# LCJebe/PCReg

Measured on AMD Instinct MI355X. Metric: KNN Gpairs/s end-to-end (search + filters + RANSAC per step; registrations/s = 1000/ms_per_step), higher is better.
Workload: dtype f32 (search: f16-split matrix-core candidates, exact f32 re-rank) / f64 (RANSAC)

## Files before the change

### include/pcreg.h

```cpp
#ifndef PCREG_H
#define PCREG_H
#include <stddef.h>
#include <stdint.h>

#ifdef __cplusplus
extern "C" {
#endif

#define PCREG_OK            0
#define PCREG_E_ARG         1
#define PCREG_E_HIP         2
#define PCREG_E_NODEVICE    3
#define PCREG_E_WORKSPACE   4

#define PCREG_KNN_MAX_K 32

#define PCREG_METRIC_SAD 0
#define PCREG_METRIC_SSD 1

typedef struct pcreg_ransac_opts {
    int32_t  minPtNum;
    int32_t  iterNum;
    double   thDist;
    double   thInlrRatio;
    int32_t  REFINE;
    int32_t  VERBOSE;
    uint64_t seed;
} pcreg_ransac_opts;

typedef struct pcreg_match_opts {
    int32_t metric;
    double  matchThreshold;
    double  maxRatio;
    int32_t unique;
    int32_t prenormalized;
    int32_t unnormalize;
    double  norm_factor;
    int32_t change_metric;
    double  metric_factor;
} pcreg_match_opts;

const char* pcreg_last_error(void);
const char* pcreg_version(void);
int  pcreg_device_count(int* count);
int  pcreg_set_device(int ordinal);
int  pcreg_device_name(char* buf, int cap);
int  pcreg_debug_set(const char* key, int value);
int  pcreg_debug_match_stats(long long out[8], int reset);
int  pcreg_debug_knn_stats(long long out[4], int reset);
int  pcreg_debug_knn_unit_stats(long long out[2], int reset);
int  pcreg_debug_knn_direct_stats(long long out[3], int reset);
int  pcreg_debug_ransac_stats(long long out[3], int reset);
int  pcreg_debug_cluster_stats(long long out[4], int reset);
int  pcreg_debug_desc_stats(long long out[10], int reset);


int pcreg_estimate_transform(const double* pts1, const double* pts2, int n, int ld,
                             double T[16], int* empty);

int pcreg_calc_dists(const double T[16], const double* pts1, const double* pts2, int n, int ld,
                     double* d);

int pcreg_ransac(const double* pts1, const double* pts2, int n, int ld,
                 const pcreg_ransac_opts* opts, const int32_t* sample_idx,
                 double T[16], int32_t* inlier_idx, int* n_inliers, int* num_success,
                 int* max_inliers, int* failed, int32_t* iter_inl, int32_t* iter_inl_ref);

int pcreg_ransac_batched(const double* pts1, const double* pts2, int total, int ld,
                         const int32_t* offsets, int B, const pcreg_ransac_opts* opts,
                         const int32_t* sample_idx, double* T, int32_t* inlier_idx,
                         int32_t* n_inliers, int32_t* num_success, int32_t* max_inliers,
                         int32_t* failed);

int pcreg_knn2_points_f32(const float* q, int Q, int ldq, const float* m, int M, int ldm,
                          int32_t* idx, float* dist);

int pcreg_match_points_f32(const float* q, int Q, int ldq, const float* m, int M, int ldm,
                           float thr_abs, float max_ratio, int unique,
                           uint32_t* pairs, int* P);

typedef struct pcreg_model pcreg_model;
int pcreg_model_create(const float* m, int M, int ldm, pcreg_model** model);
int pcreg_model_destroy(pcreg_model* model);
int pcreg_model_size(const pcreg_model* model, int* M);
int pcreg_model_match_points_f32(pcreg_model* model, const float* q, int Q, int ldq, float thr_abs, float max_ratio,
// ... 429 lines not shown
```

### pcreg_amd/_lib.py

```python
from __future__ import annotations

import ctypes as C
import os

_HERE = os.path.dirname(os.path.abspath(__file__))
LIB_PATH = os.environ.get("PCREG_LIB") or os.path.join(_HERE, "libpcreg_hip.so")

PCREG_OK, PCREG_E_ARG, PCREG_E_HIP, PCREG_E_NODEVICE, PCREG_E_WORKSPACE = 0, 1, 2, 3, 4
KNN_MAX_K = 32
METRIC_SAD, METRIC_SSD = 0, 1
LAYOUT_FEATURE_MAJOR, LAYOUT_ROW_MAJOR = 0, 1


class PcregError(RuntimeError):
    def __init__(self, code: int, msg: str):
        super().__init__(f"libpcreg_hip error {code}: {msg}")
        self.code = code


class RansacOpts(C.Structure):
    _fields_ = [("minPtNum", C.c_int32), ("iterNum", C.c_int32), ("thDist", C.c_double),
                ("thInlrRatio", C.c_double), ("REFINE", C.c_int32), ("VERBOSE", C.c_int32),
                ("seed", C.c_uint64)]


class MatchOpts(C.Structure):
    _fields_ = [("metric", C.c_int32), ("matchThreshold", C.c_double), ("maxRatio", C.c_double),
                ("unique", C.c_int32), ("prenormalized", C.c_int32), ("unnormalize", C.c_int32),
                ("norm_factor", C.c_double), ("change_metric", C.c_int32), ("metric_factor", C.c_double)]


class DescOpts(C.Structure):
    _fields_ = [("min_pts", C.c_int32), ("max_pts", C.c_int32), ("R", C.c_double), ("thVar", C.c_double * 2),
                ("k", C.c_double), ("ALIGN_POINTS", C.c_int32)]


class DevRansacResult(C.Structure):
    _fields_ = [("T", C.c_double * 16), ("n_inliers", C.c_int32), ("num_success", C.c_int32),
                ("max_inliers", C.c_int32), ("failed", C.c_int32), ("n", C.c_int32), ("winner", C.c_int32)]


SYMBOLS = [
    "pcreg_last_error", "pcreg_version", "pcreg_device_count", "pcreg_set_device", "pcreg_device_name", "pcreg_debug_set", "pcreg_debug_match_stats",
    "pcreg_debug_knn_stats", "pcreg_debug_knn_unit_stats", "pcreg_debug_knn_direct_stats", "pcreg_debug_ransac_stats", "pcreg_debug_cluster_stats", "pcreg_debug_desc_stats", "pcreg_debug_dev_model_export", "pcreg_debug_search_export",
    "pcreg_estimate_transform", "pcreg_calc_dists", "pcreg_ransac", "pcreg_ransac_batched",
    "pcreg_knn2_points_f32", "pcreg_match_points_f32", "pcreg_match_features", "pcreg_get_matches", "pcreg_desc_set_create", "pcreg_desc_set_destroy", "pcreg_desc_set_size", "pcreg_get_matches_on_sets", "pcreg_get_matches_segmented_on_sets", "pcreg_sphere_counts", "pcreg_sphere_sweep", "pcreg_sphere_model_create", "pcreg_sphere_model_destroy", "pcreg_sphere_sweep_on_model", "pcreg_final_stage_limits", "pcreg_final_stage", "pcreg_get_matches_segmented", "pcreg_get_local_points",
    "pcreg_model_create", "pcreg_model_destroy", "pcreg_model_size", "pcreg_model_match_points_f32", "pcreg_model_knn_f32", "pcreg_knn_points_f32",
    "pcreg_model_range_f32", "pcreg_range_points_f32", "pcreg_model_cluster_f32", "pcreg_cluster_points_f32",
    "pcreg_dev_model_create", "pcreg_dev_model_destroy", "pcreg_dev_model_search_workspace", "pcreg_dev_model_search_f32",
    "pcreg_dev_model_knn_workspace", "pcreg_dev_model_knn_f32", "pcreg_dev_merge_topk_f32",
    "pcreg_dev_model_range_workspace", "pcreg_dev_model_range_count_f32", "pcreg_dev_model_range_fill_f32",
    "pcreg_dev_model_cluster_workspace", "pcreg_dev_model_cluster_f32",
    "pcreg_model_score_f32", "pcreg_dev_model_score_workspace", "pcreg_dev_model_score_f32",
    "pcreg_model_refit_f32", "pcreg_dev_model_refit_workspace", "pcreg_dev_model_refit_f32",
    "pcreg_model_normals_f32", "pcreg_point_normals_f32", "pcreg_dev_model_normals_workspace", "pcreg_dev_model_normals_f32",
    "pcreg_model_refit_plane_f32", "pcreg_dev_model_refit_plane_workspace", "pcreg_dev_model_refit_plane_f32",
    "pcreg_model_denoise_f32", "pcreg_point_denoise_f32", "pcreg_dev_model_denoise_workspace", "pcreg_dev_model_denoise_f32",
    "pcreg_model_fpfh_f32", "pcreg_point_fpfh_f32", "pcreg_dev_model_fpfh_workspace", "pcreg_dev_model_fpfh_f32",
    "pcreg_model_fpfh_radius_f32", "pcreg_point_fpfh_radius_f32", "pcreg_dev_model_fpfh_radius_workspace", "pcreg_dev_model_fpfh_radius_count_f32",
    "pcreg_dev_model_fpfh_radius_f32",
    "pcreg_model_iss_f32", "pcreg_point_iss_f32", "pcreg_dev_model_iss_workspace", "pcreg_dev_model_iss_f32",
    "pcreg_model_fit_planes_f32", "pcreg_point_fit_planes_f32", "pcreg_dev_model_fit_planes_workspace", "pcreg_dev_model_fit_planes_f32",
    "pcreg_model_fit_spheres_f32", "pcreg_point_fit_spheres_f32", "pcreg_dev_model_fit_spheres_workspace", "pcreg_dev_model_fit_spheres_f32",
    "pcreg_model_fit_cylinders_f32", "pcreg_point_fit_cylinders_f32", "pcreg_dev_model_fit_cylinders_workspace", "pcreg_dev_model_fit_cylinders_f32",
    "pcreg_unique_rows3", "pcreg_aggregate_matches", "pcreg_dev_unique_rows3_workspace", "pcreg_dev_unique_rows3_f64",
    "pcreg_dev_aggregate_matches_workspace", "pcreg_dev_aggregate_matches", "pcreg_dev_estimate_transform_indexed",
    "pcreg_downsample_grid_f32", "pcreg_dev_downsample_grid_workspace", "pcreg_dev_downsample_grid_chunk", "pcreg_dev_downsample_grid_f32",
    "pcreg_ndt_create", "pcreg_ndt_destroy", "pcreg_ndt_size", "pcreg_ndt_get", "pcreg_ndt_refit_f32",
    "pcreg_dev_ndt_create", "pcreg_dev_ndt_destroy", "pcreg_dev_ndt_size", "pcreg_dev_ndt_get", "pcreg_dev_ndt_refit_workspace", "pcreg_dev_ndt_refit_f32",
    "pcreg_dev_model_match_f32", "pcreg_dev_model_match_table_f32", "pcreg_dev_match_from_table_f32",
    "pcreg_align_points_knn", "pcreg_align_points_knn_f32", "pcreg_align_points_knn_batched", "pcreg_spatial_histogram_descriptors",
    "pcreg_spatial_histogram_descriptors_f32", "pcreg_spatial_histogram_descriptors_mixed",
    "pcreg_dev_knn2_points_f32_workspace", "pcreg_dev_knn2_points_f32", "pcreg_dev_merge_top2_f32", "pcreg_dev_merge_top2_strided_f32",
    "pcreg_dev_ransac_workspace", "pcreg_dev_ransac",
    "pcreg_dev_ransac_partial", "pcreg_dev_ransac_finish", "pcreg_dev_ransac_finish_parts",
    "pcreg_dev_search_kernel_timing", "pcreg_dev_search_kernel_ms",
    "pcreg_dev_spatial_histogram_descriptors_workspace", "pcreg_dev_spatial_histogram_descriptors",
# ... 122 lines not shown
            L.pcreg_dev_model_refit_plane_workspace.argtypes = [C.c_int] * 3
            vp, i, f = C.c_void_p, C.c_int, C.c_float
            L.pcreg_dev_model_refit_plane_f32.argtypes = [vp, vp, i, i, vp, i, f, vp, i, vp, vp, vp, vp, vp, vp, vp, vp, C.c_size_t, vp]
            L.pcreg_model_refit_plane_f32.argtypes = [vp, vp, i, i, vp, i, f, i, vp, i, i, vp, vp, vp, vp, vp, vp]
        if hasattr(L, "pcreg_dev_unique_rows3_workspace"):
            for name in ("pcreg_dev_unique_rows3_workspace", "pcreg_dev_aggregate_matches_workspace"):
                getattr(L, name).restype = C.c_size_t
                getattr(L, name).argtypes = [C.c_int]
        if hasattr(L, "pcreg_dev_downsample_grid_workspace"):
            L.pcreg_dev_downsample_grid_workspace.restype = C.c_size_t
            L.pcreg_dev_downsample_grid_workspace.argtypes = [C.c_int]
            L.pcreg_dev_downsample_grid_chunk.argtypes = []
            vp, i, d = C.c_void_p, C.c_int, C.c_double
            L.pcreg_dev_downsample_grid_f32.argtypes = [vp, i, i, d, vp, i, vp, vp, vp, vp, vp, C.c_size_t, vp]
            L.pcreg_downsample_grid_f32.argtypes = [vp, i, i, d, vp, i, vp, vp, vp]
        if hasattr(L, "pcreg_dev_ndt_refit_workspace"):
            L.pcreg_dev_ndt_refit_workspace.restype = C.c_size_t
            L.pcreg_dev_ndt_refit_workspace.argtypes = [C.c_int, C.c_int]
            vp, i, d = C.c_void_p, C.c_int, C.c_double
            L.pcreg_dev_ndt_create.argtypes = [vp, i, i, d, i, vp, vp]
            L.pcreg_ndt_create.argtypes = [vp, i, i, d, i, vp]
            for name in ("pcreg_dev_ndt_destroy", "pcreg_ndt_destroy"):
                getattr(L, name).argtypes = [vp]
            for name in ("pcreg_dev_ndt_size", "pcreg_ndt_size"):
                getattr(L, name).argtypes = [vp, vp, vp]
            for name in ("pcreg_dev_ndt_get", "pcreg_ndt_get"):
                getattr(L, name).argtypes = [vp] * 7
            L.pcreg_dev_ndt_refit_f32.argtypes = [vp, vp, i, i, vp, i, i, d, vp, vp, vp, vp, vp, vp, C.c_size_t, vp]
            L.pcreg_ndt_refit_f32.argtypes = [vp, vp, i, i, vp, i, i, d, i, vp, vp, vp, vp]
        for name, args in (("pcreg_debug_knn_stats", [C.POINTER(C.c_longlong), C.c_int]),
                           ("pcreg_debug_knn_unit_stats", [C.POINTER(C.c_longlong), C.c_int]),
                           ("pcreg_debug_knn_direct_stats", [C.POINTER(C.c_longlong), C.c_int]),
                           ("pcreg_debug_ransac_stats", [C.POINTER(C.c_longlong), C.c_int]),
                           ("pcreg_debug_desc_stats", [C.POINTER(C.c_longlong), C.c_int]),
                           ("pcreg_debug_dev_model_export", [C.c_void_p] * 4 + [C.POINTER(C.c_float), C.c_void_p]),
                           ("pcreg_debug_search_export", [C.c_void_p, C.c_size_t, C.c_int, C.c_int] + [C.c_void_p] * 3)):
            if hasattr(L, name):
                getattr(L, name).argtypes = args
        _lib = L
    return _lib


def check(rc: int) -> None:
    if rc != PCREG_OK:
        raise PcregError(rc, lib().pcreg_last_error().decode(errors="replace"))
```

### pcreg_amd/csrc/api.hip

```cpp
#include "common.hpp"
#include <atomic>
#include <cstdarg>
#include <cmath>
#include <mutex>
#include <algorithm>
#include <vector>

namespace pcreg {

static thread_local char g_err[512] = "no error";
void set_error(const char* fmt, ...) {
    va_list ap; va_start(ap, fmt);
    vsnprintf(g_err, sizeof g_err, fmt, ap);
    va_end(ap);
}

constexpr int kKnnMaxK = PCREG_KNN_MAX_K;
constexpr int kKnnMaxQ = 4 << 20;
constexpr int kRangeMaxQ = 4 << 20;
constexpr int kScoreMaxQ = 4 << 20;
static std::mutex g_mu;
static int g_device_ok = -1;
static hipStream_t g_stream = nullptr;

// ... 59 lines not shown
        if (hipMalloc((void**)&c.dev, c.n * sizeof(unsigned long long)) != hipSuccess) { c.dev = nullptr; return nullptr; }
        (void)hipMemset(c.dev, 0, c.n * sizeof(unsigned long long));
    }
    return c.dev;
}
static int counters_read(const Counters& c, long long* out, int reset, int first = 0, int count = -1) {
    PCREG_ARG(out != nullptr);
    if (count < 0) count = c.n - first;
    for (int k = 0; k < count; ++k) out[k] = 0;
    if (!c.dev) return PCREG_OK;
    PCREG_HIP(hipDeviceSynchronize());
    unsigned long long h[8];
    PCREG_HIP(hipMemcpy(h, c.dev + first, count * sizeof h[0], hipMemcpyDeviceToHost));
    for (int k = 0; k < count; ++k) out[k] = (long long)h[k];
    if (reset) PCREG_HIP(hipMemset(c.dev + first, 0, count * sizeof h[0]));
    return PCREG_OK;
}
unsigned long long* match_stats_dev() { return counters_dev(g_match_stats); }
unsigned long long* knn_stats_dev() { return counters_dev(g_knn_stats); }
unsigned long long* ransac_stats_dev() { return counters_dev(g_ransac_stats); }
unsigned long long* cluster_stats_dev() { return counters_dev(g_cluster_stats); }
unsigned long long* desc_stats_dev() { return counters_dev(g_desc_stats); }
unsigned long long* knn_direct_stats_dev() { return counters_dev(g_knn_direct_stats); }
}

extern "C" {

int pcreg_debug_set(const char* key, int value) {
    static const char* const names[pcreg::kDbgCount] = {"knn_exact", "match_exact", "match_force_fallback", "ransac_fused", "ransac_nolane",
                                                        "ransac_f64score", "ransac_resident_f64", "align_times", "align_shape", "seg_debug",
                                                        "seg_batched", "seg_wave_finalize", "match_stats", "final_batch_mb", "knn_nocull",
                                                        "knn_stats", "ransac_pass2", "ransac_stats", "range_sort_cap", "cluster_noskip",
                                                        "cluster_stats", "knn_tail_cap", "score_batch_slots", "fpfh_radius_lanes", "desc_stats",
                                                        "knn_direct", "knn_direct_stats", "knn_seed_fused"};
    PCREG_ARG(key != nullptr);
    for (int k = 0; k < pcreg::kDbgCount; ++k)
        if (!strcmp(key, names[k])) { pcreg::g_debug[k].store(value, std::memory_order_relaxed); return PCREG_OK; }
    pcreg::set_error("pcreg_debug_set: unknown key '%s'", key);
    return PCREG_E_ARG;
}

int pcreg_debug_match_stats(long long out[8], int reset) { return pcreg::counters_read(pcreg::g_match_stats, out, reset); }
int pcreg_debug_knn_stats(long long out[4], int reset) { return pcreg::counters_read(pcreg::g_knn_stats, out, reset, 0, 4); }
int pcreg_debug_knn_unit_stats(long long out[2], int reset) { return pcreg::counters_read(pcreg::g_knn_stats, out, reset, 4, 2); }
int pcreg_debug_knn_direct_stats(long long out[3], int reset) { return pcreg::counters_read(pcreg::g_knn_direct_stats, out, reset); }
int pcreg_debug_ransac_stats(long long out[3], int reset) { return pcreg::counters_read(pcreg::g_ransac_stats, out, reset); }
int pcreg_debug_cluster_stats(long long out[4], int reset) { return pcreg::counters_read(pcreg::g_cluster_stats, out, reset); }
int pcreg_debug_desc_stats(long long out[10], int reset) {
    PCREG_ARG(out != nullptr);
    TRY(pcreg::counters_read(pcreg::g_desc_stats, out, reset, 0, 8));
    return pcreg::counters_read(pcreg::g_desc_stats, out + 8, reset, 8, 2);
}

const char* pcreg_last_error(void) { return g_err; }
const char* pcreg_version(void) { return "pcreg-hip 0.1 (gfx950)"; }

int pcreg_device_count(int* count) {
    PCREG_ARG(count != nullptr);
    hipError_t e = hipGetDeviceCount(count);
    if (e != hipSuccess) { *count = 0; (void)hipGetLastError(); }
    return PCREG_OK;
}

static void*  g_pin[2] = {nullptr, nullptr};
static size_t g_pin_bytes[2] = {0, 0};
static hipEvent_t g_pairs_ev = nullptr;

int pcreg_set_device(int ordinal) {
    std::lock_guard<std::mutex> lock(g_mu);
    int count = 0;
    if (hipGetDeviceCount(&count) != hipSuccess || count <= 0) { set_error("no HIP device available"); (void)hipGetLastError(); return PCREG_E_NODEVICE; }
    PCREG_ARG(ordinal >= 0 && ordinal < count);
    scratch().release_all();
    if (g_stream) { (void)hipStreamDestroy(g_stream); g_stream = nullptr; }
    if (g_pairs_ev) { (void)hipEventDestroy(g_pairs_ev); g_pairs_ev = nullptr; }
    for (int k = 0; k < 2; ++k) if (g_pin[k]) { (void)hipHostFree(g_pin[k]); g_pin[k] = nullptr; g_pin_bytes[k] = 0; }
    g_device_ok = -1;
    PCREG_HIP(hipSetDevice(ordinal));
    return ensure_device();
// ... 2551 lines not shown
```

### pcreg_amd/csrc/common.hpp

```cpp
#pragma once
#include <cstdlib>
#include <hip/hip_runtime.h>
#include <cstdint>
#include <cstdio>
#include <cstring>
#include <algorithm>
#include <string>
#include "../../include/pcreg.h"

namespace pcreg {

void set_error(const char* fmt, ...);
int  ensure_device();

#define PCREG_HIP(call)                                                                  \
    do {                                                                                 \
        hipError_t e__ = (call);                                                         \
        if (e__ != hipSuccess) {                                                         \
            ::pcreg::set_error("%s failed: %s (%s:%d)", #call, hipGetErrorString(e__),   \
                               __FILE__, __LINE__);                                      \
            return PCREG_E_HIP;                                                          \
        }                                                                                \
    } while (0)

#define PCREG_ARG(cond)                                                                  \
    do {                                                                                 \
        if (!(cond)) {                                                                   \
            ::pcreg::set_error("bad argument: %s (%s:%d)", #cond, __FILE__, __LINE__);   \
            return PCREG_E_ARG;                                                          \
        }                                                                                \
    } while (0)

struct Scratch {
    static constexpr int kSlots = 24;
    void*  ptr[kSlots]  = {};
    size_t size[kSlots] = {};
    int get(int slot, size_t bytes, void** out);
    void release_all();
};
// ... 8 lines not shown
        return rc;
    }
};

enum DebugKey {
    kDbgKnnExact = 0,
    kDbgMatchExact,
    kDbgMatchForceFallback,
    kDbgRansacFused,
    kDbgRansacNoLane,
    kDbgRansacF64Score,
    kDbgRansacResidentF64,
    kDbgAlignTimes,
    kDbgAlignShape,
    kDbgSegDebug,
    kDbgSegBatched,
    kDbgSegWaveFinalize,
    kDbgMatchStats,
    kDbgFinalBatchMB,
    kDbgKnnNoCull,
    kDbgKnnStats,
    kDbgRansacPass2,
    kDbgRansacStats,
    kDbgRangeSortCap,
    kDbgClusterNoSkip,
    kDbgClusterStats,
    kDbgKnnTailCap,
    kDbgScoreBatchSlots,
    kDbgFpfhRadiusLanes,
    kDbgDescStats,
    kDbgKnnDirect,
    kDbgKnnDirectStats,
    kDbgKnnSeedFused,
    kDbgCount
};
int debug_flag(DebugKey k);
unsigned long long* match_stats_dev();
unsigned long long* knn_stats_dev();
unsigned long long* knn_direct_stats_dev();
unsigned long long* ransac_stats_dev();
unsigned long long* cluster_stats_dev();
unsigned long long* desc_stats_dev();
#ifdef PCREG_EXPERIMENTS
static inline int pcreg_env_int(const char* name, int dflt) { const char* e = getenv(name); return e ? atoi(e) : dflt; }
static inline const char* pcreg_env_str(const char* name) { return getenv(name); }
#define PCREG_EXP_ENV(name, dflt) pcreg_env_int(name, dflt)
#define PCREG_EXP_STR(name) pcreg_env_str(name)
#else
#define PCREG_EXP_ENV(name, dflt) (dflt)
#define PCREG_EXP_STR(name) ((const char*)nullptr)
#endif

static inline size_t align_up(size_t x, size_t a) { return (x + a - 1) / a * a; }

struct WsWalk {
    char* base; size_t off = 0;
    explicit WsWalk(void* b) : base((char*)b) {}
    void* take_bytes(size_t bytes) { void* p = base ? base + off : nullptr; off += bytes; return p; }
    template <class T> T* take(size_t count, size_t align = 256) { return (T*)take_bytes(align_up(count * sizeof(T), align)); }
    size_t bytes() const { return off; }
};

template <typename T>
static int upload_cols(const T* host, int n, int ld, int cols, T* dev, hipStream_t st) {
    if (n <= 0 || cols <= 0) return PCREG_OK;
    if (ld == n) { PCREG_HIP(hipMemcpyAsync(dev, host, sizeof(T) * (size_t)n * cols, hipMemcpyHostToDevice, st)); }
    else PCREG_HIP(hipMemcpy2DAsync(dev, sizeof(T) * (size_t)n, host, sizeof(T) * (size_t)ld, sizeof(T) * (size_t)n, cols, hipMemcpyHostToDevice, st));
    return PCREG_OK;
}

struct RansacDims { int n_cap; int iters; int B; };

size_t ransac_workspace_bytes(int iters, int B, int n_cap);
// ... 217 lines not shown
```

### pcreg_amd/csrc/ransac.hip

```cpp
#include "common.hpp"
#include "moments.hpp"
#include "wave_math.hpp"
#include <cfloat>
#include <cstddef>
#include <cstdio>
#include <cstdlib>

namespace pcreg {
namespace {

constexpr int kBlock = 256;
constexpr int kWavesPerBlock = 4;
constexpr int HB = 4;

struct RansacArgs {
    const double* p1; const double* p2; int ld;
    const int32_t* offsets;
    const int32_t* n_dev;
    int n_cap; int iters; int m;
    double thDist; double ratio; int refine; unsigned long long seed;
    const int32_t* sample_idx;
    int hpw;
    int hyp0g;
    double* TF;
// ... 1324 lines not shown
                cnt += __popcll(b[s]);                                                                             \
                if (EMIT) {                                                               \
                    asm volatile("v_writelane_b32 %0, %1, %2" : "+v"(mine_lo) : "s"((int)(unsigned)b[s]), "n"(s)); \
                    asm volatile("v_writelane_b32 %0, %1, %2" : "+v"(mine_hi) : "s"((int)(unsigned)(b[s] >> 32)), "n"(s)); \
                }                                                                                                  \
            }                                                                                                      \
            if (lane == 0) s_cnt[wave][(H) - h0] += cnt;                                                           \
            if (EMIT && lane < kSS)                            \
                sa.masks[(size_t)(H) * sa.nslots_cap + (size_t)pb * (kSPts / 64) + wave * kSS + lane] =            \
                    ((unsigned long long)(unsigned)mine_hi << 32) | (unsigned)mine_lo;                             \
        }
        PCREG_ROW_LOAD(RA, h0)
        PCREG_ROW_WAIT(RA);
        for (int h = h0; h < h1; h += 2) {
            PCREG_ROW_LOAD(RB, h + 1)
            PCREG_SCORE_HYP(h, RA)
            PCREG_ROW_WAIT(RB); PCREG_ROW_LOAD(RA, h + 2)
            if (h + 1 < h1) { PCREG_SCORE_HYP(h + 1, RB) }
            PCREG_ROW_WAIT(RA);
        }
#undef PCREG_SCORE_HYP
#undef PCREG_ROW_WAIT
#undef PCREG_ROW_LOAD
    }
    __syncthreads();
    for (int hl = threadIdx.x; hl < h1 - h0; hl += kSW * 64) {
        int c = 0;
#pragma unroll
        for (int w = 0; w < kSW; ++w) c += s_cnt[w][hl];
        if (acc) { if (c) atomicAdd(&acc[h0 + hl], c); } else sa.part[(size_t)blockIdx.x * a.iters + h0 + hl] = c;
    }
}


__device__ __forceinline__ void rs_load_block(const StagedArgs& sa, const float* __restrict__ x32, int base, int n, float (&q)[kSS][6]) {
    const int lane = threadIdx.x & 63;
#pragma unroll
    for (int s = 0; s < kSS; ++s) {
        const int i = base + s * 64 + lane;
        const bool act = i < n;
        const int ii = act ? i : 0;
#pragma unroll
        for (int c = 0; c < 6; ++c) q[s][c] = x32[(size_t)c * sa.n32 + ii];
        if (!act) q[s][0] = __builtin_nanf("");
    }
}
__device__ __forceinline__ int rs_block_count(const StagedArgs& sa, const float* __restrict__ x32, const int32_t* __restrict__ perm,
                                              int base, int n, const float (&q)[kSS][6], const float (&T)[12], float thlo, float thhi,
                                              int h) {
    const RansacArgs& a = sa.a;
    const int lane = threadIdx.x & 63;
    unsigned long long b[kSS], band = 0ull;
#pragma unroll
    for (int s = 0; s < kSS; ++s) {
        const float d = sqdist32(q[s], T);
        b[s] = __ballot(d < thlo);
        band |= __ballot(d <= thhi) ^ b[s];
    }
    if (band != 0ull && !PCREG_NOBAND(sa)) {
        double T64[12];
#pragma unroll
        for (int k = 0; k < 12; ++k) T64[k] = a.TF[(size_t)h * 12 + k];
#pragma unroll 1
        for (int s = 0; s < kSS; ++s) {
            const int i = base + s * 64 + lane;
            const bool act = i < n;
// ... 1477 lines not shown
            double tv = 0.0;
#pragma unroll
            for (int e = 0; e < 12; ++e) if (e == j * 4 + k) tv = T[e];
            v = (j < 3) ? tv : (k == 3 ? 1.0 : 0.0);
        }
        s_S[k + 4 * j] = v;
        if (T_step) T_step[(size_t)bl * 16 + k + 4 * j] = v;
    }
    __builtin_amdgcn_fence(__ATOMIC_ACQ_REL, "wavefront"); __builtin_amdgcn_wave_barrier();
    if (lane < 16) {
        const int r = lane & 3, c = lane >> 2;
        const double* Ti = T_in + (size_t)bl * 16;
        const double v = ((Ti[r] * s_S[4 * c] + Ti[r + 4] * s_S[1 + 4 * c]) + Ti[r + 8] * s_S[2 + 4 * c]) + Ti[r + 12] * s_S[3 + 4 * c];
        T_out[(size_t)bl * 16 + r + 4 * c] = ok ? v : 0.0;
    }
    if (lane == 0) empty[bl] = ok ? 0 : 1;
}

__global__ void calc_dists_kernel(const double* T16, const double* p1, const double* p2, int n, int ld, double* d) {
    double T[12];
#pragma unroll
    for (int j = 0; j < 3; ++j)
#pragma unroll
        for (int k = 0; k < 4; ++k) T[j * 4 + k] = T16[k + 4 * j];
    Pts<false> P{p1, p2, ld, nullptr, n};
    for (int i = blockIdx.x * blockDim.x + threadIdx.x; i < n; i += gridDim.x * blockDim.x) {
        double q[6]; P.load(i, q);
        d[i] = sqdist(q, T);
    }
}

}

static bool staged_pays(int n_cap, int iters) { return n_cap >= 4096 || (n_cap >= kStagedMinN && (long long)n_cap * iters >= 20000000LL); }
static bool bounded_pays(int n_cap, int iters) {
    const double full_us = (double)n_cap * (double)iters / 2.4e6, bounded_us = 1.4 * (double)((n_cap + kBBlk - 1) / kBBlk) + 30.0;
    return full_us > 1.1 * bounded_us;
}
static size_t staged_slots_cap(int n_cap) { return (size_t)((n_cap + kSPts - 1) / kSPts) * (kSPts / 64); }
static size_t staged_chunks_cap(int n_cap) { return (staged_slots_cap(n_cap) + kMomSlots - 1) / kMomSlots; }
struct RansacWs { double* TF; int32_t* cnt1; int32_t* cnt2; unsigned char* has; double* msc; StagedArgs sa; };
static RansacWs ransac_ws_layout(int iters, int B, int n_cap, void* base, size_t* bytes) {
    const size_t h = (size_t)iters * (size_t)B;
    const int nc = B == 1 ? n_cap : 0;
    const size_t slots = staged_slots_cap(nc);
    WsWalk w(base);
    RansacWs s{};
    StagedArgs& sa = s.sa;
    s.TF = w.take<double>(h * 12);
    s.cnt1 = w.take<int32_t>(h); s.cnt2 = w.take<int32_t>(h);
    s.has = w.take<unsigned char>(h); s.msc = w.take<double>(h * 16);
    sa.T1 = w.take<double>(h * 12); sa.mom = w.take<double>(h * 27);
    sa.part = w.take<int32_t>(h * kSMaxPB);
    sa.v1 = w.take<unsigned char>(h); sa.pass1 = w.take<unsigned char>(h); sa.v2 = w.take<unsigned char>(h);
    sa.cert = w.take<unsigned char>(h); sa.dense = w.take<unsigned char>(h);
    sa.bounds = (double*)w.take_bytes(256);
    sa.n_rec_blocks = (int)((slots * 64 + 255) / 256);
    sa.bpart = w.take<double>((size_t)sa.n_rec_blocks * 4);
    sa.sel_ctr = w.take_bytes(512);
    sa.certq = w.take<double>(h * 2);
    if (nc >= kStagedMinN) {
        sa.nslots_cap = (int)slots;
        sa.masks = w.take<unsigned long long>(h * slots);
        sa.rec = w.take<double>(slots * 64 * kRec + 32);
        sa.mpart = w.take<double>(staged_chunks_cap(nc) * h * 15);
        sa.pass_list = w.take<int32_t>(h);
        sa.dig = w.take<uint4>(slots * 2 * 256);
        sa.n_pass = (int32_t*)w.take_bytes(256);
        sa.n32 = (int)slots * 64;
        sa.c32 = w.take<float>((size_t)sa.n32 * 6);
// ... 59 lines not shown
        const int c = n_cap <= kHyp32Classes[0] ? 0 : 1;
        a.n_lo = -1; a.n_hi = std::min(n_cap, kHyp32Classes[c]);
        const int nw = kHyp32Waves[c], per_block = hpw * nw;
        const dim3 grid((o.iterNum + per_block - 1) / per_block, B);
        const int rc = nw == 8 ? launch_hyp32<8>(a, grid, hyp32_lds_bytes(a.n_hi, nw), st) : launch_hyp32<16>(a, grid, hyp32_lds_bytes(a.n_hi, nw), st);
        if (rc != PCREG_OK) return rc;
        const int lo = a.n_hi;
        if (n_cap > lo) {
            a.n_lo = lo; a.n_hi = -1;
            const int pb4 = hpw * kWavesPerBlock;
            hipLaunchKernelGGL(ransac_hyp_kernel, dim3((o.iterNum + pb4 - 1) / pb4, B), dim3(kBlock), 0, st, a);
        }
    } else if (B == 1 && !offsets && staged_pays(n_cap, o.iterNum) && !debug_flag(kDbgRansacFused)) {
        StagedArgs sa = lay.sa;
        sel_ctr = sa.sel_ctr;
        sa.use_lane = a.refine && !debug_flag(kDbgRansacNoLane);
        sa.use_f32 = !debug_flag(kDbgRansacF64Score);
#ifdef PCREG_EXPERIMENTS
        sa.noband = PCREG_EXP_ENV("PCREG_RANSAC_NOBAND", 0);
#endif
        int pb = (n_cap + kSPts - 1) / kSPts; if (pb > kSMaxPB) pb = kSMaxPB; if (pb < 1) pb = 1;
        sa.pb = pb;
        int hpw = (int)((total + 250LL * kTW - 1) / (250LL * kTW));
        if (hpw < 1) hpw = 1;
        if (hpw > 16) hpw = 16;
        a.hpw = hpw;
        sa.a = a;
        const int it = o.iterNum;
        const dim3 sgrid(pb, (it + kSChunk - 1) / kSChunk);
        const int n_fit = (it + 255) / 256;
        hipLaunchKernelGGL(rs_stage1_kernel, dim3((unsigned)(n_fit + sa.n_rec_blocks)), dim3(256), 0, st, sa, n_fit);
        const int n_t32 = (it + 255) / 256, n_dig = sa.use_lane ? (int)staged_slots_cap(n_cap) * 2 : 0;
        hipLaunchKernelGGL(rs_stage2_kernel, dim3((unsigned)(n_t32 + n_dig)), dim3(256), 0, st, sa, (const double*)sa.T1, sa.T32a, n_t32, sa.dig);
        if (sa.use_f32) {
            if (sa.use_lane)
                hipLaunchKernelGGL(rs_score32_kernel<true>, sgrid, dim3(kSW * 64), 0, st, sa, (const double*)sa.T1, (const float*)sa.T32a, (const unsigned char*)sa.v1, (int32_t*)nullptr);
            else
                hipLaunchKernelGGL(rs_score32_kernel<false>, sgrid, dim3(kSW * 64), 0, st, sa, (const double*)sa.T1, (const float*)sa.T32a, (const unsigned char*)sa.v1, (int32_t*)nullptr);
        } else if (sa.use_lane) {
            hipLaunchKernelGGL(rs_score_kernel<true>, sgrid, dim3(kSW * 64), 0, st, sa, (const double*)sa.T1, (const unsigned char*)sa.v1);
        } else {
            hipLaunchKernelGGL(rs_score_kernel<false>, sgrid, dim3(kSW * 64), 0, st, sa, (const double*)sa.T1, (const unsigned char*)sa.v1);
        }
        hipLaunchKernelGGL(rs_pass1_kernel, dim3((it + 255) / 256), dim3(256), 0, st, sa);
        if (a.refine) {
            if (sa.use_lane)
                hipLaunchKernelGGL(rs_moments_mfma_kernel, dim3((it + kMmWaves * kMmRows - 1) / (kMmWaves * kMmRows), (unsigned)staged_chunks_cap(n_cap)), dim3(kMmWaves * 64), 0, st, sa,
                                   (const uint4*)sa.dig, (const unsigned long long*)sa.masks);
            hipLaunchKernelGGL(rs_moments_kernel, dim3((it + hpw * kTW - 1) / (hpw * kTW)), dim3(kTBlock), 0, st, sa);
            hipLaunchKernelGGL(rs_fit2_kernel, dim3((it + 63) / 64), dim3(64), 0, st, sa);
            fold_finish = !part && n_cap <= kSelBlocks * kSelPerThread * kSelThreads;
            const int p2mode = debug_flag(kDbgRansacPass2);
            const bool bounded = fold_finish && sa.use_f32 && !iter_inl_ref && p2mode != 1 && (p2mode == 2 || bounded_pays(n_cap, it));
            if (bounded) {
                const int S = std::min(kBSeeds, it), nbc = (n_cap + kBBlk - 1) / kBBlk;
                const int n_seed_wg = (S * nbc + 3) / 4, n_ord_wg = (n_cap + 255) / 256;
                unsigned long long* stats = ransac_stats_dev();
                hipLaunchKernelGGL(rs_bprep_kernel, dim3((unsigned)(n_seed_wg + n_ord_wg)), dim3(256), 0, st, sa, n_seed_wg, S, nbc);
                hipLaunchKernelGGL(rs_bscatter_kernel, dim3((unsigned)n_ord_wg), dim3(256), 0, st, sa);
#ifdef PCREG_EXPERIMENTS
                const int dbg = PCREG_EXP_ENV("PCREG_RANSAC_DEBUG", 0), chunk = PCREG_EXP_ENV("PCREG_RANSAC_BCHUNK", kBChunk);
                unsigned long long* kst = dbg ? ((BCtr*)sa.bctr)->stats : stats;
                if (chunk == 8) hipLaunchKernelGGL(rs_bounded_kernel<8>, dim3((unsigned)((it + 7) / 8)), dim3(64), 0, st, sa, kst);
                else if (chunk == 2) hipLaunchKernelGGL(rs_bounded_kernel<2>, dim3((unsigned)((it + 1) / 2)), dim3(64), 0, st, sa, kst);
                else hipLaunchKernelGGL(rs_bounded_kernel<kBChunk>, dim3((unsigned)((it + kBChunk - 1) / kBChunk)), dim3(64), 0, st, sa, kst);
                if (dbg) {
                    unsigned long long u[3] = {0, 0, 0};
                    PCREG_HIP(hipMemcpyAsync(u, kst, sizeof u, hipMemcpyDeviceToHost, st));
                    PCREG_HIP(hipStreamSynchronize(st));
                    fprintf(stderr, "[pcreg] ransac bounded pass 2: iters=%d n_cap=%d chunk=%d (refit, block) units scanned %llu of %llu (%.4f)\n", it, n_cap,
                            chunk == 8 || chunk == 2 ? chunk : kBChunk, u[1], u[2], u[2] ? (double)u[1] / (double)u[2] : 0.0);
                }
#else
                hipLaunchKernelGGL(rs_bounded_kernel<kBChunk>, dim3((unsigned)((it + kBChunk - 1) / kBChunk)), dim3(64), 0, st, sa, stats);
#endif
            } else if (sa.use_f32)
                hipLaunchKernelGGL(rs_score32_kernel<false>, sgrid, dim3(kSW * 64), 0, st, sa, (const double*)a.TF, (const float*)sa.T32b, (const unsigned char*)sa.v2,
                                   fold_finish ? a.cnt2 : (int32_t*)nullptr);
            else
                hipLaunchKernelGGL(rs_score_kernel<false>, sgrid, dim3(kSW * 64), 0, st, sa, (const double*)a.TF, (const unsigned char*)sa.v2);
            if (fold_finish) { sel_fin.part = sa.use_f32 ? nullptr : sa.part; sel_fin.v2 = sa.v2; sel_fin.pb = sa.pb; }
            else hipLaunchKernelGGL(rs_finish_kernel, dim3((it + 255) / 256), dim3(256), 0, st, sa);
        }
    } else {
        int hpw = (int)((total + 250LL * kTW - 1) / (250LL * kTW));
        if (hpw < 1) hpw = 1;
        if (hpw > 16) hpw = 16;
        a.hpw = hpw;
        int per_block = hpw * kTW;
        dim3 grid((o.iterNum + per_block - 1) / per_block, B);
        hipLaunchKernelGGL(ransac_hyp_tiled_kernel, grid, dim3(kTBlock), 0, st, a);
    }
    PCREG_HIP(hipGetLastError());
    if (sel_ctr && !part && n_cap <= kSelBlocks * kSelPerThread * kSelThreads) {
        int per_block = 4 * kSelThreads;
        if ((n_cap + per_block - 1) / per_block > kSelBlocks) per_block = ((n_cap + kSelBlocks - 1) / kSelBlocks + kSelThreads - 1) / kSelThreads * kSelThreads;
        const int nb = std::max(1, (n_cap + per_block - 1) / per_block);
        hipLaunchKernelGGL(ransac_select_multi_kernel, dim3(nb), dim3(kSelThreads), 0, st, a, out, inlier_idx, (SelCtr*)sel_ctr, per_block, sel_fin);
    }
    else if (n_cap >= 8192) hipLaunchKernelGGL(ransac_select_kernel<1024>, dim3(B), dim3(1024), 0, st, a, out, inlier_idx, part);
    else hipLaunchKernelGGL(ransac_select_kernel<kBlock>, dim3(B), dim3(kBlock), 0, st, a, out, inlier_idx, part);
    PCREG_HIP(hipGetLastError());
    if (iter_inl) PCREG_HIP(hipMemcpyAsync(iter_inl, a.cnt1, h * sizeof(int32_t), hipMemcpyDeviceToDevice, st));
    if (iter_inl_ref) PCREG_HIP(hipMemcpyAsync(iter_inl_ref, a.cnt2, h * sizeof(int32_t), hipMemcpyDeviceToDevice, st));
    return PCREG_OK;
}

int launch_ransac(const double* p1, const double* p2, int ld, const int32_t* offsets, const int32_t* n_dev,
                  int n_cap, int B, const pcreg_ransac_opts& o, const int32_t* sample_idx_dev,
                  pcreg_dev_ransac_result* out, int32_t* inlier_idx, int32_t* iter_inl, int32_t* iter_inl_ref,
                  void* ws, size_t ws_bytes, hipStream_t st) {
    return launch_ransac_impl(p1, p2, ld, offsets, n_dev, n_cap, B, o, sample_idx_dev, out, inlier_idx, iter_inl, iter_inl_ref,
                              ws, ws_bytes, st, 0, nullptr);
}

// ... 73 lines not shown
```

Baseline: 142,600.

## Add hypothesis-per-lane RANSAC scoring kernel with LDS-staged points and ballot masks

Adds rs_hscore_kernel, where each lane owns one RANSAC hypothesis and the workgroup stages 512 points in shared memory. Each lane tests every staged point with an inline-asm f32 transform-distance routine, builds inlier bitmasks from low/high band thresholds via ballots, and resolves ambiguous band points with an exact f64 check. The kernel is meant to replace rs_score32_kernel when the workgroup count is large enough, for both the first scoring pass and the pass-2 rescoring. It aims to raise data reuse and cut per-point work. The trade-offs are higher register pressure and a divergent f64 fallback loop.

```diff
diff --git a/include/pcreg.h b/include/pcreg.h
--- a/include/pcreg.h
+++ b/include/pcreg.h
@@ -51,6 +51,7 @@
 int  pcreg_debug_knn_unit_stats(long long out[2], int reset);
 int  pcreg_debug_knn_direct_stats(long long out[3], int reset);
 int  pcreg_debug_ransac_stats(long long out[3], int reset);
+int  pcreg_debug_ransac_score_stats(long long out[2], int reset);
 int  pcreg_debug_cluster_stats(long long out[4], int reset);
 int  pcreg_debug_desc_stats(long long out[10], int reset);
 
diff --git a/pcreg_amd/_lib.py b/pcreg_amd/_lib.py
--- a/pcreg_amd/_lib.py
+++ b/pcreg_amd/_lib.py
@@ -42,7 +42,7 @@
 
 SYMBOLS = [
     "pcreg_last_error", "pcreg_version", "pcreg_device_count", "pcreg_set_device", "pcreg_device_name", "pcreg_debug_set", "pcreg_debug_match_stats",
-    "pcreg_debug_knn_stats", "pcreg_debug_knn_unit_stats", "pcreg_debug_knn_direct_stats", "pcreg_debug_ransac_stats", "pcreg_debug_cluster_stats", "pcreg_debug_desc_stats", "pcreg_debug_dev_model_export", "pcreg_debug_search_export",
+    "pcreg_debug_knn_stats", "pcreg_debug_knn_unit_stats", "pcreg_debug_knn_direct_stats", "pcreg_debug_ransac_stats", "pcreg_debug_ransac_score_stats", "pcreg_debug_cluster_stats", "pcreg_debug_desc_stats", "pcreg_debug_dev_model_export", "pcreg_debug_search_export",
     "pcreg_estimate_transform", "pcreg_calc_dists", "pcreg_ransac", "pcreg_ransac_batched",
     "pcreg_knn2_points_f32", "pcreg_match_points_f32", "pcreg_match_features", "pcreg_get_matches", "pcreg_desc_set_create", "pcreg_desc_set_destroy", "pcreg_desc_set_size", "pcreg_get_matches_on_sets", "pcreg_get_matches_segmented_on_sets", "pcreg_sphere_counts", "pcreg_sphere_sweep", "pcreg_sphere_model_create", "pcreg_sphere_model_destroy", "pcreg_sphere_sweep_on_model", "pcreg_final_stage_limits", "pcreg_final_stage", "pcreg_get_matches_segmented", "pcreg_get_local_points",
     "pcreg_model_create", "pcreg_model_destroy", "pcreg_model_size", "pcreg_model_match_points_f32", "pcreg_model_knn_f32", "pcreg_knn_points_f32",
@@ -231,6 +231,7 @@
                            ("pcreg_debug_knn_unit_stats", [C.POINTER(C.c_longlong), C.c_int]),
                            ("pcreg_debug_knn_direct_stats", [C.POINTER(C.c_longlong), C.c_int]),
                            ("pcreg_debug_ransac_stats", [C.POINTER(C.c_longlong), C.c_int]),
+                           ("pcreg_debug_ransac_score_stats", [C.POINTER(C.c_longlong), C.c_int]),
                            ("pcreg_debug_desc_stats", [C.POINTER(C.c_longlong), C.c_int]),
                            ("pcreg_debug_dev_model_export", [C.c_void_p] * 4 + [C.POINTER(C.c_float), C.c_void_p]),
                            ("pcreg_debug_search_export", [C.c_void_p, C.c_size_t, C.c_int, C.c_int] + [C.c_void_p] * 3)):
diff --git a/pcreg_amd/csrc/api.hip b/pcreg_amd/csrc/api.hip
--- a/pcreg_amd/csrc/api.hip
+++ b/pcreg_amd/csrc/api.hip
@@ -115,7 +115,7 @@
                                                         "seg_batched", "seg_wave_finalize", "match_stats", "final_batch_mb", "knn_nocull",
                                                         "knn_stats", "ransac_pass2", "ransac_stats", "range_sort_cap", "cluster_noskip",
                                                         "cluster_stats", "knn_tail_cap", "score_batch_slots", "fpfh_radius_lanes", "desc_stats",
-                                                        "knn_direct", "knn_direct_stats", "knn_seed_fused"};
+                                                        "knn_direct", "knn_direct_stats", "knn_seed_fused", "ransac_score"};
     PCREG_ARG(key != nullptr);
     for (int k = 0; k < pcreg::kDbgCount; ++k)
         if (!strcmp(key, names[k])) { pcreg::g_debug[k].store(value, std::memory_order_relaxed); return PCREG_OK; }
@@ -128,6 +128,11 @@
 int pcreg_debug_knn_unit_stats(long long out[2], int reset) { return pcreg::counters_read(pcreg::g_knn_stats, out, reset, 4, 2); }
 int pcreg_debug_knn_direct_stats(long long out[3], int reset) { return pcreg::counters_read(pcreg::g_knn_direct_stats, out, reset); }
 int pcreg_debug_ransac_stats(long long out[3], int reset) { return pcreg::counters_read(pcreg::g_ransac_stats, out, reset); }
+int pcreg_debug_ransac_score_stats(long long out[2], int reset) {
+    PCREG_ARG(out != nullptr);
+    for (int k = 0; k < 2; ++k) out[k] = reset ? pcreg::g_ransac_score_launches[k].exchange(0) : pcreg::g_ransac_score_launches[k].load();
+    return PCREG_OK;
+}
 int pcreg_debug_cluster_stats(long long out[4], int reset) { return pcreg::counters_read(pcreg::g_cluster_stats, out, reset); }
 int pcreg_debug_desc_stats(long long out[10], int reset) {
     PCREG_ARG(out != nullptr);
diff --git a/pcreg_amd/csrc/common.hpp b/pcreg_amd/csrc/common.hpp
--- a/pcreg_amd/csrc/common.hpp
+++ b/pcreg_amd/csrc/common.hpp
@@ -5,6 +5,7 @@
 #include <cstdio>
 #include <cstring>
 #include <algorithm>
+#include <atomic>
 #include <string>
 #include "../../include/pcreg.h"
 
@@ -79,6 +80,7 @@
     kDbgKnnDirect,
     kDbgKnnDirectStats,
     kDbgKnnSeedFused,
+    kDbgRansacScore,
     kDbgCount
 };
 int debug_flag(DebugKey k);
@@ -86,6 +88,7 @@
 unsigned long long* knn_stats_dev();
 unsigned long long* knn_direct_stats_dev();
 unsigned long long* ransac_stats_dev();
+extern std::atomic<long long> g_ransac_score_launches[2];
 unsigned long long* cluster_stats_dev();
 unsigned long long* desc_stats_dev();
 #ifdef PCREG_EXPERIMENTS
diff --git a/pcreg_amd/csrc/ransac.hip b/pcreg_amd/csrc/ransac.hip
--- a/pcreg_amd/csrc/ransac.hip
+++ b/pcreg_amd/csrc/ransac.hip
@@ -1380,6 +1380,153 @@
     }
 }
 
+__device__ __forceinline__ void push_bit(unsigned& own, unsigned long long ballot);
+__device__ __forceinline__ float sqdist32v(const float4& q, const float2& r, const float (&T)[12]) {
+    float tx, ty, tz, d;
+    asm("v_fma_f32 %0, %9, %12, %19\n\t"
+        "v_fma_f32 %1, %9, %15, %20\n\t"
+        "v_fma_f32 %2, %9, %18, %21\n\t"
+        "v_fma_f32 %0, %8, %11, %0\n\t"
+        "v_fma_f32 %1, %8, %14, %1\n\t"
+        "v_fma_f32 %2, %8, %17, %2\n\t"
+        "v_fma_f32 %0, %7, %10, %0\n\t"
+        "v_fma_f32 %1, %7, %13, %1\n\t"
+        "v_fma_f32 %2, %7, %16, %2\n\t"
+        "v_sub_f32 %0, %4, %0\n\t"
+        "v_sub_f32 %1, %5, %1\n\t"
+        "v_sub_f32 %2, %6, %2\n\t"
+        "v_mul_f32 %3, %0, %0\n\t"
+        "v_fma_f32 %3, %1, %1, %3\n\t"
+        "v_fma_f32 %3, %2, %2, %3"
+        : "=&v"(tx), "=&v"(ty), "=&v"(tz), "=&v"(d)
+        : "v"(q.x), "v"(q.y), "v"(q.z), "v"(q.w), "v"(r.x), "v"(r.y),
+          "v"(T[0]), "v"(T[1]), "v"(T[2]), "v"(T[3]), "v"(T[4]), "v"(T[5]), "v"(T[6]), "v"(T[7]), "v"(T[8]),
+          "v"(T[9]), "v"(T[10]), "v"(T[11]));
+    return d;
+}
+constexpr int kHPts = 512, kHW = 4, kHWords = kHPts / 32;
+typedef unsigned rs_u32x16 __attribute__((ext_vector_type(16)));
+static_assert(kHWords == 16 && kSPts % kHPts == 0, "a lane's words are one rs_u32x16; the blocks tile rs_score32_kernel's");
+template <bool EMIT>
+__global__ __launch_bounds__(kHW * 64) void rs_hscore_kernel(StagedArgs sa, const double* __restrict__ TT,
+                                                             const float* __restrict__ T32,
+                                                             const unsigned char* __restrict__ valid,
+                                                             int32_t* __restrict__ acc ) {
+    const RansacArgs& a = sa.a;
+    __shared__ float4 s_rec[kHPts * 2];
+    const int n = staged_n(a);
+    const int h = blockIdx.y * (kHW * 64) + threadIdx.x;
+    const int hc = min(h, a.iters - 1);
+    const bool live = h < a.iters && valid[hc] != 0;
+    float T[12], thlo, thhi;
+    {
+        const float4* rp = (const float4*)(T32 + (size_t)hc * 16);
+        const float4 r0 = rp[0], r1 = rp[1], r2 = rp[2], r3 = rp[3];
+        T[0] = r0.x; T[1] = r0.y; T[2] = r0.z; T[3] = r0.w; T[4] = r1.x; T[5] = r1.y; T[6] = r1.z; T[7] = r1.w;
+        T[8] = r2.x; T[9] = r2.y; T[10] = r2.z; T[11] = r2.w; thlo = r3.x; thhi = r3.y;
+    }
+    const double th = a.thDist;
+    int cnt = 0;
+    const int nblk = (n + kSPts - 1) / kSPts * (kSPts / kHPts);
+    for (int pb = blockIdx.x; pb < nblk; pb += gridDim.x) {
+        const int base = pb * kHPts;
+        uint4* mrow = (uint4*)(sa.masks + (size_t)hc * sa.nslots_cap + (size_t)pb * (kHPts / 64));
+        if (base >= n) {
+            if (EMIT && live) { const uint4 z = make_uint4(0u, 0u, 0u, 0u); mrow[0] = z; mrow[1] = z; mrow[2] = z; mrow[3] = z; }
+            continue;
+        }
+        if (pb != (int)blockIdx.x) __syncthreads();
+#pragma unroll
+        for (int k = 0; k < kHPts / (kHW * 64); ++k) {
+            const int r = k * (kHW * 64) + threadIdx.x, i = base + r;
+            const bool act = i < n;
+            const int ii = act ? i : 0;
+            float q[6];
+#pragma unroll
+            for (int c = 0; c < 6; ++c) q[c] = sa.c32[(size_t)c * sa.n32 + ii];
+            if (!act) q[0] = __builtin_nanf("");
+            s_rec[2 * r] = make_float4(q[0], q[1], q[2], q[3]);
+            *(float2*)&s_rec[2 * r + 1] = make_float2(q[4], q[5]);
+        }
+        __syncthreads();
+        rs_u32x16 lo, hi;
+#define PCREG_HREAD(W, G) _Pragma("unroll") for (int e = 0; e < 4; ++e) {                                              \
+            const float4* rp_ = s_rec + (W) * 64 + ((G) * 4 + e) * 2; nA[e] = rp_[0]; nB[e] = *(const float2*)(rp_ + 1); }
+#pragma unroll 1
+        for (int w = 0; w < kHWords; ++w) {
+            unsigned l = 0u, u = 0u;
+            float4 A[4]; float2 B[4];
+            { float4 nA[4]; float2 nB[4]; PCREG_HREAD(w, 7)
+#pragma unroll
+              for (int e = 0; e < 4; ++e) { A[e] = nA[e]; B[e] = nB[e]; } }
+#pragma unroll
+            for (int g = 7; g >= 0; --g) {
+                float4 nA[4]; float2 nB[4];
+                if (g > 0) { PCREG_HREAD(w, g - 1) }
+#pragma unroll
+                for (int e = 3; e >= 0; --e) {
+                    const float d = sqdist32v(A[e], B[e], T);
+                    push_bit(l, __ballot(d < thlo));
+                    push_bit(u, __ballot(d <= thhi));
+                }
+                if (g > 0) {
+#pragma unroll
+                    for (int e = 0; e < 4; ++e) { A[e] = nA[e]; B[e] = nB[e]; }
+                }
+            }
+            lo[w] = l; hi[w] = u;
+        }
+#undef PCREG_HREAD
+        unsigned left = 0u;
+#pragma unroll
+        for (int k = 0; k < kHWords; ++k) left |= lo[k] ^ hi[k];
+        if (!live || PCREG_NOBAND(sa)) left = 0u;
+        if (__ballot(left != 0u) != 0ull) {
+            double T64[12];
+            if (left != 0u) {
+#pragma unroll
+                for (int k = 0; k < 12; ++k) T64[k] = TT[(size_t)h * 12 + k];
+            }
+#pragma unroll 1
+            while (__ballot(left != 0u) != 0ull) {
+                if (left != 0u) {
+                    int w = 0; unsigned x = 0u;
+#pragma unroll
+                    for (int k = kHWords - 1; k >= 0; --k) { const unsigned xk = lo[k] ^ hi[k]; w = xk ? k : w; x = xk ? xk : x; }
+                    const int bit = __builtin_ctz(x);
+                    const int i = base + w * 32 + bit;
+                    const bool act = i < n;
+                    const int ii = act ? i : 0;
+                    double p[6];
+#pragma unroll
+                    for (int c = 0; c < 3; ++c) { p[c] = a.p1[ii + (size_t)c * a.ld]; p[3 + c] = a.p2[ii + (size_t)c * a.ld]; }
+                    const bool in = (sqdist(p, T64) < th) & act;
+                    const unsigned m = 1u << bit;
+                    left = 0u;
+#pragma unroll
+                    for (int k = 0; k < kHWords; ++k) {
+                        const unsigned nl = in ? lo[k] | m : lo[k] & ~m;
+                        lo[k] = k == w ? nl : lo[k];
+                        hi[k] = k == w ? ((hi[k] & ~m) | (nl & m)) : hi[k];
+                        left |= lo[k] ^ hi[k];
+                    }
+                }
+            }
+        }
+        if (live) {
+#pragma unroll
+            for (int k = 0; k < kHWords; ++k) cnt += __popc(lo[k]);
+            if (EMIT) {
+#pragma unroll
+                for (int k = 0; k < 4; ++k) mrow[k] = make_uint4(lo[4 * k], lo[4 * k + 1], lo[4 * k + 2], lo[4 * k + 3]);
+            }
+        }
+    }
+    if (h < a.iters) {
+        if (acc) { if (cnt) atomicAdd(&acc[h], cnt); } else sa.part[(size_t)blockIdx.x * a.iters + h] = cnt;
+    }
+}
+
 
 __device__ __forceinline__ void rs_load_block(const StagedArgs& sa, const float* __restrict__ x32, int base, int n, float (&q)[kSS][6]) {
     const int lane = threadIdx.x & 63;
@@ -2923,10 +3070,16 @@
 
 }
 
+std::atomic<long long> g_ransac_score_launches[2];
+
 static bool staged_pays(int n_cap, int iters) { return n_cap >= 4096 || (n_cap >= kStagedMinN && (long long)n_cap * iters >= 20000000LL); }
 static bool bounded_pays(int n_cap, int iters) {
     const double full_us = (double)n_cap * (double)iters / 2.4e6, bounded_us = 1.4 * (double)((n_cap + kBBlk - 1) / kBBlk) + 30.0;
     return full_us > 1.1 * bounded_us;
+}
+static bool hscore_pays(int n_cap, int iters, bool emit) {
+    const long long wgs = (long long)std::min(kSMaxPB, (n_cap + kHPts - 1) / kHPts) * ((iters + kHW * 64 - 1) / (kHW * 64));
+    return emit && wgs >= 1280;
 }
 static size_t staged_slots_cap(int n_cap) { return (size_t)((n_cap + kSPts - 1) / kSPts) * (kSPts / 64); }
 static size_t staged_chunks_cap(int n_cap) { return (staged_slots_cap(n_cap) + kMomSlots - 1) / kMomSlots; }
@@ -3052,7 +3205,21 @@
         hipLaunchKernelGGL(rs_stage1_kernel, dim3((unsigned)(n_fit + sa.n_rec_blocks)), dim3(256), 0, st, sa, n_fit);
         const int n_t32 = (it + 255) / 256, n_dig = sa.use_lane ? (int)staged_slots_cap(n_cap) * 2 : 0;
         hipLaunchKernelGGL(rs_stage2_kernel, dim3((unsigned)(n_t32 + n_dig)), dim3(256), 0, st, sa, (const double*)sa.T1, sa.T32a, n_t32, sa.dig);
-        if (sa.use_f32) {
+        const int smode = debug_flag(kDbgRansacScore);
+        const bool hscore = sa.use_f32 && smode != 1 && (smode == 2 || hscore_pays(n_cap, it, sa.use_lane != 0));
+        const bool hscore2 = sa.use_f32 && smode != 1 && (smode == 2 || hscore_pays(n_cap, it, false));
+        StagedArgs sh = sa;
+        sh.pb = std::max(1, std::min(kSMaxPB, (n_cap + kHPts - 1) / kHPts));
+        const dim3 hgrid(sh.pb, (it + kHW * 64 - 1) / (kHW * 64));
+        const bool count_launches = debug_flag(kDbgRansacStats) != 0;
+        if (hscore) {
+            if (count_launches) g_ransac_score_launches[0]++;
+            if (sa.use_lane)
+                hipLaunchKernelGGL(rs_hscore_kernel<true>, hgrid, dim3(kHW * 64), 0, st, sh, (const double*)sa.T1, (const float*)sa.T32a, (const unsigned char*)sa.v1, (int32_t*)nullptr);
+            else
+                hipLaunchKernelGGL(rs_hscore_kernel<false>, hgrid, dim3(kHW * 64), 0, st, sh, (const double*)sa.T1, (const float*)sa.T32a, (const unsigned char*)sa.v1, (int32_t*)nullptr);
+        } else if (sa.use_f32) {
+            if (count_launches) g_ransac_score_launches[1]++;
             if (sa.use_lane)
                 hipLaunchKernelGGL(rs_score32_kernel<true>, sgrid, dim3(kSW * 64), 0, st, sa, (const double*)sa.T1, (const float*)sa.T32a, (const unsigned char*)sa.v1, (int32_t*)nullptr);
             else
@@ -3062,7 +3229,7 @@
         } else {
             hipLaunchKernelGGL(rs_score_kernel<false>, sgrid, dim3(kSW * 64), 0, st, sa, (const double*)sa.T1, (const unsigned char*)sa.v1);
         }
-        hipLaunchKernelGGL(rs_pass1_kernel, dim3((it + 255) / 256), dim3(256), 0, st, sa);
+        hipLaunchKernelGGL(rs_pass1_kernel, dim3((it + 255) / 256), dim3(256), 0, st, hscore ? sh : sa);
         if (a.refine) {
             if (sa.use_lane)
                 hipLaunchKernelGGL(rs_moments_mfma_kernel, dim3((it + kMmWaves * kMmRows - 1) / (kMmWaves * kMmRows), (unsigned)staged_chunks_cap(n_cap)), dim3(kMmWaves * 64), 0, st, sa,
@@ -3094,13 +3261,18 @@
 #else
                 hipLaunchKernelGGL(rs_bounded_kernel<kBChunk>, dim3((unsigned)((it + kBChunk - 1) / kBChunk)), dim3(64), 0, st, sa, stats);
 #endif
-            } else if (sa.use_f32)
+            } else if (hscore2) {
+                if (count_launches) g_ransac_score_launches[0]++;
+                hipLaunchKernelGGL(rs_hscore_kernel<false>, hgrid, dim3(kHW * 64), 0, st, sh, (const double*)a.TF, (const float*)sa.T32b, (const unsigned char*)sa.v2,
+                                   fold_finish ? a.cnt2 : (int32_t*)nullptr);
+            } else if (sa.use_f32) {
+                if (count_launches) g_ransac_score_launches[1]++;
                 hipLaunchKernelGGL(rs_score32_kernel<false>, sgrid, dim3(kSW * 64), 0, st, sa, (const double*)a.TF, (const float*)sa.T32b, (const unsigned char*)sa.v2,
                                    fold_finish ? a.cnt2 : (int32_t*)nullptr);
-            else
+            } else
                 hipLaunchKernelGGL(rs_score_kernel<false>, sgrid, dim3(kSW * 64), 0, st, sa, (const double*)a.TF, (const unsigned char*)sa.v2);
             if (fold_finish) { sel_fin.part = sa.use_f32 ? nullptr : sa.part; sel_fin.v2 = sa.v2; sel_fin.pb = sa.pb; }
-            else hipLaunchKernelGGL(rs_finish_kernel, dim3((it + 255) / 256), dim3(256), 0, st, sa);
+            else hipLaunchKernelGGL(rs_finish_kernel, dim3((it + 255) / 256), dim3(256), 0, st, hscore2 ? sh : sa);
         }
     } else {
         int hpw = (int)((total + 250LL * kTW - 1) / (250LL * kTW));
```

Result: faster. 144,000, median of 6 (+1.0%).
